# bwfbowen/muax

Hardware: AMD Instinct MI355X
Metric: batched act() env-steps/sec at num_simulations=50 (higher is better)
Workload: dtype f32; 1 GPU; cartpole: 4096 roots/GPU, obs 4, MLP embed 8, A=2, support 10, num_simulations=50, dirichlet 0.25/0.3, tiebreak=threefry, temperature 1; roots_per_gpu=4096, num_simulations=50, parallelism=roots sharded x1, no collective, backend=none (one rank), launcher=none

## Files before the change

### muax_amd/csrc/mz_fused.cuh

```cuda
#pragma once
#include "mz_spec.cuh"

#pragma clang fp contract(off)

namespace mz {

#ifdef MZ_PROFILE
#define MZ_TICK(slot)                                  \
  do {                                                 \
    uint64_t now_ = __builtin_amdgcn_s_memtime();      \
    prof_acc[slot] += now_ - prof_t;                   \
    prof_t = now_;                                     \
  } while (0)
#define MZ_TICKW(slot)                                 \
  do {                                                 \
    asm volatile("s_waitcnt vmcnt(0) lgkmcnt(0)" ::: "memory"); \
    MZ_TICK(slot);                                     \
  } while (0)
#else
#define MZ_TICK(slot) do {} while (0)
#define MZ_TICKW(slot) do {} while (0)
#endif

constexpr int kMaxSims = 256;
// ... 778 lines not shown
    for (int t = 0; t < C::ES; ++t) {
      int k = j + 16 * t;
      float acc = 0.0f;
      {
        const int kc = k < E ? k : 0;
        int i = 0;
        for (; i + 4 <= p.obs_dim; i += 4) {
          float o4[4], w4[4];
#pragma unroll
          for (int q = 0; q < 4; ++q) {
            o4[q] = ob[i + q];
            w4[q] = p.repr_w[(i + q) * E + kc];
          }
#pragma unroll
          for (int q = 0; q < 4; ++q) acc = __builtin_fmaf(o4[q], w4[q], acc);
        }
        for (; i < p.obs_dim; ++i) acc = __builtin_fmaf(ob[i], p.repr_w[i * E + kc], acc);
        acc = acc + p.repr_b[kc];
      }
      s[t] = k < E ? acc : 0.0f;
    }
    row_min_max_normalize<E>(s, j);
  }
  float v0, pl0;
  nets.predict(s, j, support, p.F, v0, pl0);
  uint32_t inv_bits = 0;
  if (p.invalid != nullptr) {
#pragma unroll
    for (int a = 0; a < A; ++a) inv_bits |= p.invalid[(size_t)r * A + a] ? (1u << a) : 0u;
  }
  int ncons = 0;
  int root_jw;
  {
    float lg, pq[1];
    if constexpr (!C::GUMBEL) {
      float x[1] = {pl0}, pr[1];
      row_softmax<A>(x, j, pr);
      float nz = (p.dirichlet_noise != nullptr && j < A) ? p.dirichlet_noise[(size_t)r * A + j] : 0.0f;
      float keep = 1.0f - p.dirichlet_fraction;
      float noisy = keep * pr[0] + p.dirichlet_fraction * nz;
      lg = log_pos(fmaxf(noisy, kFltTiny));
      if (p.invalid != nullptr) {
        float mx = row_max<4>(j < A ? lg : -INFINITY);
        lg = ((inv_bits >> j) & 1u) ? kFltLowest : lg - mx;
      }
      float lx[1] = {lg};
      row_softmax<A>(lx, j, pq);
    } else {
      lg = pl0;
      if (inv_bits != 0) {
        float mx = row_max<4>(j < A ? lg : -INFINITY);
        lg = ((inv_bits >> j) & 1u) ? kFltLowest : lg - mx;
      }
      pq[0] = 0.0f;
      float g;
      if (p.gumbel != nullptr) {
        g = j < A ? p.gumbel[(size_t)r * A + j] : 0.0f;
      } else {
        uint32_t x0, x1;
        bool second;
        bits_block(p.global_batch * (uint64_t)A, rg * (uint64_t)A + (uint64_t)(j < A ? j : 0), x0, x1, second);
        threefry2x32(p.k_gumbel[0], p.k_gumbel[1], x0, x1);
        g = p.gumbel_scale * gumbel_from_bits(second ? x1 : x0);
      }
      if (j < A) {
        tree[C::GUM0 + j] = g;
        tree[C::off_logit(j)] = lg;
      }
      ncons = min(p.max_considered, A - __builtin_popcount(inv_bits));
    }
    if (j < A) tree[C::off_prob(j)] = pq[0];
    if (ex && j < A) p.t_children_prior_logits[(size_t)r * N * A + j] = lg;
    if (j == 0) {
      itree[C::HDR0] = 1;
      tree[C::HDR0 + 1] = v0;
      if constexpr (C::RAW_OK) tree[C::HDR0 + 3] = v0;
      p.root_value[r] = v0;
      if (ex) p.t_raw_values[(size_t)r * N] = v0;
    }
#pragma unroll
    for (int t = 0; t < C::ES; ++t)
      if (j + 16 * t < E) {
        if constexpr (C::EMB_LDS) tree[C::EMB0 + j + 16 * t] = s[t];
        else gemb[j + 16 * t] = s[t];
      }
    float prob[A], val[A], rew[A], dis[A], sc[A];
    int vis[A];
#pragma unroll
    for (int a = 0; a < A; ++a) {
      prob[a] = tree[C::off_prob(a)];
      val[a] = 0.0f; vis[a] = 0; rew[a] = 0.0f; dis[a] = p.discount;
    }
    int cidx[A], best, child;
    bool safe;
    if constexpr (!C::GUMBEL) {
      float rcp1[A];
#pragma unroll
      for (int a = 0; a < A; ++a) rcp1[a] = 1.0f;
      puct_scores<A>(v0, tbl[2], prob, val, vis, rew, dis, rcp1, sc);
    } else {
      float logit[A], gum[A];
#pragma unroll
      for (int a = 0; a < A; ++a) {
        logit[a] = tree[C::off_logit(a)];
        gum[a] = tree[C::GUM0 + a];
      }
      gumbel_scores<A, C::QT>(true, v0, v0, logit, val, vis, rew, dis, gum, p.visit_table[(size_t)ncons * S],
                              inv_bits, sc);
    }
#pragma unroll
    for (int a = 0; a < A; ++a) {
      cidx[a] = -1;
      sc[a] = ((inv_bits >> a) & 1u) ? -INFINITY : sc[a];
    }
    decide<A, C::TB>(sc, cidx, best, child, safe);
    root_jw = jump_word(0, best, 0, !safe);
    if (j == 0) {
#pragma unroll
      for (int a = 0; a < A; ++a) tree[C::off_score(a)] = sc[a];
      itree[C::JUMP] = root_jw;
    }
  }

  int depth_total = 0;
  int pref_parent = 0;
  float pre[C::ES];
#pragma unroll
  for (int t = 0; t < C::ES; ++t) pre[t] = 0.0f;
  if constexpr (!C::EMB_LDS) {
#pragma unroll
    for (int t = 0; t < C::ES; ++t) pre[t] = s[t];
  }
  MZ_TICKW(12);

  for (int sim = 0; sim < S; ++sim) {
    MZ_TICK(0);
    int cv_next = 0;
    if constexpr (C::GUMBEL) cv_next = p.visit_table[(size_t)ncons * S + (sim + 1 < S ? sim + 1 : S - 1)];
    int parent, action, dP;
    int next = -1;
    parent = root_jw & 0xfff;
    action = (root_jw >> 12) & 0xf;
    dP = (root_jw >> 16) & 0xff;
    int depth = dP + 1;
    bool rare = depth > max_depth;
    if constexpr (C::TB) rare = rare || root_jw < 0;
    if (__builtin_amdgcn_ballot_w64(rare) != 0) {
      uint32_t fk0 = 0, fk1 = 0, fs0 = 0, fs1 = 0;
      int fk_level = -1;
      int jw = root_jw;
      for (;;) {
        parent = jw & 0xfff;
        action = (jw >> 12) & 0xf;
        dP = (jw >> 16) & 0xff;
        if constexpr (C::TB) {
          if (jw < 0 && dP + 1 <= max_depth) {
            const int* ndi = itree + __umul24((unsigned)parent, (unsigned)NS);
            if (fk_level < 0) {
              uint32_t x0, x1;
              bool second;
              bits_block(2 * p.global_batch, 2 * rg + (uint64_t)(j & 1), x0, x1, second);
              threefry2x32(p.sim_keys[sim][0], p.sim_keys[sim][1], x0, x1);
              uint32_t word = second ? x1 : x0;
              fk0 = bcast_u<0>(word);
              fk1 = bcast_u<1>(word);
              fk_level = 0;
            }
#ifdef MZ_PROFILE
            prof_acc[14] += 1;
            prof_acc[15] += (uint64_t)(dP + 1 - fk_level);
#endif
            while (fk_level <= dP) {
              uint32_t x0 = (uint32_t)(j & 1), x1 = 2u + (uint32_t)(j & 1);
              threefry2x32(fk0, fk1, x0, x1);
              fk0 = bcast_u<0>(x0); fk1 = bcast_u<1>(x0);
              fs0 = bcast_u<0>(x1); fs1 = bcast_u<1>(x1);
              fk_level += 1;
            }
            constexpr int NB = (A + 1) / 2;
            const int jb = j % NB;
            uint32_t x0 = (uint32_t)jb, x1 = (NB + jb < A) ? (uint32_t)(NB + jb) : 0u;
            threefry2x32(fs0, fs1, x0, x1);
            int cidx[A];
            float score[A];
            C::load_cidx(ndi, cidx);
            StaticFor<0, A>::run([&](auto ic) {
              constexpr int a = decltype(ic)::value;
              const uint32_t bits = bcast_u<(a % NB)>(a < NB ? x0 : x1);
              score[a] = __int_as_float(ndi[C::off_score(a)]) + 1e-7f * uniform_from_bits(bits);
            });
            int best = 0, bn = cidx[0];
            float bs = score[0];
#pragma unroll
            for (int a = 1; a < A; ++a) {
              bool take = score[a] > bs;
              bs = take ? score[a] : bs;
              best = take ? a : best;
              bn = take ? cidx[a] : bn;
            }
            action = best;
            next = bn;
            if (bn >= 0 && dP + 1 < max_depth) {
              jw = itree[__umul24((unsigned)bn, (unsigned)NS) + C::JUMP];
              next = -1;
              continue;
            }
          }
        }
        break;
      }
      depth = dP + 1;
      if (depth > max_depth) {
        depth = max_depth;
        const int* pb = C::PH ? gpath + (size_t)parent * C::PATHW : itree + __umul24((unsigned)parent, (unsigned)NS) + C::PATH0;
        const int e = depth - 1;
        const int ent = (pb[(e * C::ENTRY_BITS) >> 5] >> ((e * C::ENTRY_BITS) & 31)) & ((1 << C::ENTRY_BITS) - 1);
        parent = ent & ((1 << C::ENTRY_ACT_SHIFT) - 1);
        action = ent >> C::ENTRY_ACT_SHIFT;
        next = C::load_cidx1(itree + __umul24((unsigned)parent, (unsigned)NS), action);
      }
    }
    depth_total += depth;
    MZ_TICK(1);
    const bool fresh = next < 0;
    const int newn = fresh ? sim + 1 : next;

    float sp[C::ES];
#pragma unroll
    for (int t = 0; t < C::ES; ++t)
      if constexpr (C::EMB_LDS) {
        const int jc = j + 16 * t < E ? j + 16 * t : E - 1;
        const float v = tree[__umul24((unsigned)parent, (unsigned)NS) + C::EMB0 + jc];
        sp[t] = (j + 16 * t < E) ? v : 0.0f;
      } else {
        float v = pre[t];
        if (parent != pref_parent && j + 16 * t < E) v = gemb[(size_t)parent * E + j + 16 * t];
        sp[t] = (j + 16 * t < E) ? v : 0.0f;
      }
    float* nn = tree + __umul24((unsigned)newn, (unsigned)NS);
    int* nni = reinterpret_cast<int*>(nn);
    const unsigned po = __umul24((unsigned)parent, (unsigned)NS);
    const int vis_old = nni[C::HDR0];
    int ppw[C::PATHS];
#pragma unroll
    for (int t = 0; t < C::PATHS; ++t) {
      const int wi = j + 16 * t < C::PATHW ? j + 16 * t : 0;
      if constexpr (C::PH) ppw[t] = gpath[(size_t)parent * C::PATHW + wi];
      else ppw[t] = itree[po + C::PATH0 + wi];
    }
    float reward, value, pil, pprob;
    float ns[C::ES];
    nets.forward(sp, action, j, support, p.F, p.pred_on_parent != 0, reward, value, pil, pprob, ns);
    MZ_TICK(2);
    {
      const int vis = vis_old + 1;
      if (j < A) {
        nn[C::off_prob(j)] = pprob;
        if constexpr (C::GUMBEL) nn[C::off_logit(j)] = pil;
      }
#pragma unroll
      for (int t = 0; t < C::ES; ++t)
        if (j + 16 * t < E) {
          if constexpr (C::EMB_LDS) nn[C::EMB0 + j + 16 * t] = ns[t];
          else gemb[(size_t)newn * E + j + 16 * t] = ns[t];
        }
      if (j == 0) {
        nni[C::HDR0] = vis;
        nn[C::HDR0 + 1] = value;
        if constexpr (C::RAW_OK) nn[C::HDR0 + 3] = value;
        C::store_cidx(itree + po, action, newn);
        tree[po + C::off_rew(action)] = reward;
      }
      if (fresh) {
        const int e = depth - 1;
        const int sh = (e * C::ENTRY_BITS) & 31;
        const int ent = parent | (action << C::ENTRY_ACT_SHIFT);
#pragma unroll
        for (int t = 0; t < C::PATHS; ++t) {
          const int wi = j + 16 * t;
          int w = ppw[t];
          w = (wi == ((e * C::ENTRY_BITS) >> 5))
                  ? (int)(((unsigned)w & ~(((1u << C::ENTRY_BITS) - 1u) << sh)) | ((unsigned)ent << sh))
                  : w;
          if (wi < C::PATHW) {
            if constexpr (C::PH) gpath[(size_t)newn * C::PATHW + wi] = w;
            else nni[C::PATH0 + wi] = w;
          }
        }
      }
      if (ex) {
        size_t o = (size_t)r * N + newn;
        if (j < A) p.t_children_prior_logits[o * A + j] = pil;
        if (j == 0) {
          p.t_raw_values[o] = value;
          p.t_parents[o] = parent;
          p.t_action_from_parent[o] = action;
        }
      }
    }

    MZ_TICK(4);
    {
      int wmax;
      {
        const int d0 = __builtin_amdgcn_readlane(depth, 0), d1 = __builtin_amdgcn_readlane(depth, 16);
        const int d2 = __builtin_amdgcn_readlane(depth, 32), d3 = __builtin_amdgcn_readlane(depth, 48);
        int m01, m23;
        asm("s_max_i32 %0, %1, %2" : "=s"(m01) : "s"(d0), "s"(d1) : "scc");
        asm("s_max_i32 %0, %1, %2" : "=s"(m23) : "s"(d2), "s"(d3) : "scc");
        asm("s_max_i32 %0, %1, %2" : "=s"(wmax) : "s"(m01), "s"(m23) : "scc");
      }
      float G = value;
      float carry_v = value;
      int carry_n = -1;
      int carry_j = 0;
      for (int c = wmax >> 4; c >= 0; --c) {
        const int e = 16 * c + j;
        const bool valid = e <= depth;
        const bool isleaf = e == depth;
        const bool edge = e < depth;
        int pn, pa;
        {
          const int ec = e < depth - 1 ? e : 0;
          const int widx = (ec * C::ENTRY_BITS) >> 5;
          const int slot_c = ((16 * c * C::ENTRY_BITS) >> 5) >> 4;
          int psrc = ppw[0];
#pragma unroll
          for (int t = 1; t < C::PATHS; ++t) psrc = (slot_c == t) ? ppw[t] : psrc;
          const int pword = __builtin_amdgcn_ds_bpermute(4 * ((lane & ~15) + (widx & 15)), psrc);
          const int ent = (pword >> ((ec * C::ENTRY_BITS) & 31)) & ((1 << C::ENTRY_BITS) - 1);
          pn = ent & ((1 << C::ENTRY_ACT_SHIFT) - 1);
          pa = ent >> C::ENTRY_ACT_SHIFT;
          pn = e == depth - 1 ? parent : pn;
          pa = e == depth - 1 ? action : pa;
          pn = isleaf ? newn : pn;
          pa = isleaf ? 0 : pa;
          pn = valid ? pn : 0;
        }
        MZ_TICKW(6);
        float* nd = tree + __umul24((unsigned)pn, (unsigned)NS);
        int* ndi = reinterpret_cast<int*>(nd);
        const int cnt = ndi[C::HDR0];
        const float pv = nd[C::HDR0 + 1];
        float prob[A], val[A], rew[A], dis[A];
        int vis[A], cidx[A];
        C::load_cidx(ndi, cidx);
        C::load_vis(ndi, vis);
#pragma unroll
        for (int a = 0; a < A; ++a) {
          prob[a] = nd[C::off_prob(a)];
          val[a] = nd[C::off_val(a)];
          rew[a] = nd[C::off_rew(a)];
          dis[a] = p.discount;
        }
        int jch[A];
#pragma unroll
        for (int a = 0; a < A; ++a)
          jch[a] = itree[__umul24((unsigned)(cidx[a] < 0 ? 0 : cidx[a]), (unsigned)NS) + C::JUMP];
        const int nvis = edge ? cnt + 1 : cnt;
        const float2 tn_rc = *reinterpret_cast<const float2*>(tbl + 2 * (valid ? nvis : 0));
        float rcp1[A];
#pragma unroll
        for (int a = 0; a < A; ++a) {
          vis[a] = (edge && pa == a) ? vis[a] + 1 : vis[a];
          rcp1[a] = tbl[2 * (vis[a] + 1) + 1];
        }
        MZ_TICKW(7);
        float re = rew[0];
#pragma unroll
        for (int a = 1; a < A; ++a) re = (pa == a) ? rew[a] : re;
        re = edge ? re : 0.0f;
        const float ge = edge ? p.discount : 1.0f;
        const int kstart = min(15, wmax - 16 * c);
        float Gt = ge * G;
#define MZ_GSTEP_TXT "s_nop 1\n\tv_mul_f32_dpp %0, %1, %2 row_shl:1 row_mask:0xf bank_mask:0xf\n\tv_add_f32 %1, %0, %3\n\t"
#define MZ_GSTEP4 \
  asm volatile(MZ_GSTEP_TXT MZ_GSTEP_TXT MZ_GSTEP_TXT MZ_GSTEP_TXT : "+v"(Gt), "+v"(G) : "v"(ge), "v"(re));
        if (kstart >= 12) { MZ_GSTEP4 }
        if (kstart >= 8) { MZ_GSTEP4 }
        if (kstart >= 4) { MZ_GSTEP4 }
        float sc[A];
        constexpr bool kFill = !C::GUMBEL && A == 2;
        if constexpr (kFill) {
          float d0, d1, x0, x1, q0, q1, r0, r1;
#define MZ_GSTEP_BODY "v_mul_f32_dpp %[Gt], %[G], %[ge] row_shl:1 row_mask:0xf bank_mask:0xf\n\tv_add_f32 %[G], %[Gt], %[re]\n\t"
          asm volatile(
              "v_add_u32 %[d0], 1, %[v0]\n\tv_add_u32 %[d1], 1, %[v1]\n\tv_mul_f32 %[x0], %[tn], %[p0]\n\t" MZ_GSTEP_BODY
              "v_cvt_f32_i32 %[d0], %[d0]\n\tv_cvt_f32_i32 %[d1], %[d1]\n\tv_mul_f32 %[x1], %[tn], %[p1]\n\t" MZ_GSTEP_BODY
              "v_mul_f32 %[q0], %[x0], %[y0]\n\tv_mul_f32 %[q1], %[x1], %[y1]\n\tv_fma_f32 %[r0], -%[q0], %[d0], %[x0]\n\t" MZ_GSTEP_BODY
              "v_fma_f32 %[r1], -%[q1], %[d1], %[x1]\n\tv_fma_f32 %[s0], %[r0], %[y0], %[q0]\n\tv_fma_f32 %[s1], %[r1], %[y1], %[q1]\n\t"
              MZ_GSTEP_BODY
              : [Gt] "+v"(Gt), [G] "+v"(G), [d0] "=&v"(d0), [d1] "=&v"(d1), [x0] "=&v"(x0), [x1] "=&v"(x1), [q0] "=&v"(q0),
                [q1] "=&v"(q1), [r0] "=&v"(r0), [r1] "=&v"(r1), [s0] "=&v"(sc[0]), [s1] "=&v"(sc[A - 1])
              : [ge] "v"(ge), [re] "v"(re), [tn] "v"(tn_rc.x), [p0] "v"(prob[0]), [p1] "v"(prob[A - 1]), [v0] "v"(vis[0]),
                [v1] "v"(vis[A - 1]), [y0] "v"(rcp1[0]), [y1] "v"(rcp1[A - 1]));
#undef MZ_GSTEP_BODY
        } else {
          MZ_GSTEP4
        }
#undef MZ_GSTEP4
#undef MZ_GSTEP_TXT
        const float Gown = G;
        G = bcast<0>(G);
        MZ_TICKW(8);
        const float newv = div_small(pv * (float)cnt + Gown, (float)cnt + 1.0f, tn_rc.y);
        float childv = __int_as_float(__builtin_amdgcn_update_dpp(
            __float_as_int(carry_v), __float_as_int(newv), 0x101 , 0xf, 0xf, false));
        childv = (e == depth - 1) ? value : childv;
        carry_v = bcast<0>(newv);
        const int next_pn = __builtin_amdgcn_update_dpp(carry_n, pn, 0x101, 0xf, 0xf, false);
        carry_n = bcast_i<0>(pn);
#pragma unroll
        for (int a = 0; a < A; ++a) val[a] = (edge && pa == a) ? childv : val[a];
        const float nval = edge ? newv : pv;
        MZ_TICKW(9);
        if constexpr (!C::GUMBEL) {
          puct_scores<A, true, kFill>(nval, tn_rc.x, prob, val, vis, rew, dis, rcp1, sc);
#pragma unroll
          for (int a = 0; a < A; ++a)
            sc[a] = (pn == 0 && ((inv_bits >> a) & 1u)) ? -INFINITY : sc[a];
        } else {
          float logit[A], gum[A];
#pragma unroll
          for (int a = 0; a < A; ++a) {
            logit[a] = nd[C::off_logit(a)];
            gum[a] = tree[C::GUM0 + a];
          }
          gumbel_scores<A, C::QT>(pn == 0, nval, C::RAW_OK ? nd[C::HDR0 + C::HDRW - 1] : 0.0f, logit, val, vis, rew, dis, gum, cv_next,
                                  pn == 0 ? inv_bits : 0u, sc);
        }
        MZ_TICKW(10);
        int best, child;
        bool safe;
        decide<A, C::TB>(sc, cidx, best, child, safe);
        const bool inherit0 = valid && safe && child >= 0 && !isleaf && child == next_pn;
        int jchild = jch[0];
#pragma unroll
        for (int a = 1; a < A; ++a) jchild = (best == a) ? jch[a] : jchild;
        const int jwd0 = jump_word(pn, best, e, !safe);
        int jwd = (safe && child >= 0 && !inherit0) ? jchild : jwd0;
        int done = inherit0 ? 0 : -1;
#define MZ_JSCAN(d)                                                                              \
  {                                                                                              \
    const int jn = __builtin_amdgcn_update_dpp(0, jwd, 0x100 + d, 0xf, 0xf, true);               \
    const int dn = __builtin_amdgcn_update_dpp(0, done, 0x100 + d, 0xf, 0xf, true);              \
    jwd = (jwd & done) | (jn & ~done);                                                           \
    done = done | dn;                                                                            \
  }
        MZ_JSCAN(1) MZ_JSCAN(2) MZ_JSCAN(4) MZ_JSCAN(8)
#undef MZ_JSCAN
        jwd = (jwd & done) | (carry_j & ~done);
        carry_j = bcast_i<0>(jwd);
        MZ_TICKW(11);
        if (valid) {
#pragma unroll
          for (int a = 0; a < A; ++a) nd[C::off_score(a)] = sc[a];
          ndi[C::JUMP] = jwd;
          ndi[C::HDR0] = nvis;
          nd[C::HDR0 + 1] = nval;
          float cvn = val[0];
          int cin = vis[0];
#pragma unroll
          for (int a = 1; a < A; ++a) {
            cvn = (pa == a) ? val[a] : cvn;
            cin = (pa == a) ? vis[a] : cin;
          }
          nd[C::off_val(pa)] = cvn;
          C::store_vis(ndi, pa, cin);
        }
      }
      root_jw = carry_j;
      if constexpr (!C::EMB_LDS) {
        pref_parent = carry_j & 0xfff;
#pragma unroll
        for (int t = 0; t < C::ES; ++t)
          pre[t] = (j + 16 * t < E) ? gemb[(size_t)pref_parent * E + j + 16 * t] : 0.0f;
      }
    }
    MZ_TICK(5);
  }

  if constexpr (C::GUMBEL) {
    float logit[A], val[A], rew[A], dis[A], gum[A], qv[A], sc[A], x[A], w[A];
    int vis[A], sumv, cv = 0;
#pragma unroll
    for (int a = 0; a < A; ++a) {
      val[a] = tree[C::off_val(a)];
      vis[a] = itree[C::ST0 + C::STW * a + 2];
      rew[a] = tree[C::off_rew(a)];
      dis[a] = p.discount;
      logit[a] = tree[C::off_logit(a)];
      gum[a] = tree[C::GUM0 + a];
      cv = max(cv, vis[a]);
    }
    const float nval = tree[C::HDR0 + 1], raw = C::RAW_OK ? tree[C::HDR0 + C::HDRW - 1] : 0.0f;
    gumbel_scores<A, C::QT>(true, nval, raw, logit, val, vis, rew, dis, gum, cv, inv_bits, sc);
    qtransform_inlane<A, C::QT>(nval, raw, logit, val, vis, rew, dis, qv, sumv);
    int best = 0;
    float bs = sc[0], mx = logit[0] + qv[0];
#pragma unroll
    for (int a = 0; a < A; ++a) {
      x[a] = logit[a] + qv[a];
      mx = fmaxf(mx, x[a]);
      bool take = a > 0 && sc[a] > bs;
      bs = take ? sc[a] : bs;
      best = take ? a : best;
    }
    if (inv_bits != 0) {
#pragma unroll
      for (int a = 0; a < A; ++a) x[a] = ((inv_bits >> a) & 1u) ? kFltLowest : x[a] - mx;
    }
    softmax_inlane<A>(x, w);
    if (j < A) {
      float mine = w[0];
#pragma unroll
      for (int a = 1; a < A; ++a) mine = (j == a) ? w[a] : mine;
      p.action_weights[(size_t)r * A + j] = mine;
    }
    if (j == 0) {
      p.action[r] = best;
      if (p.search_value) p.search_value[r] = nval;
      if (p.depth_sum) p.depth_sum[r] = depth_total;
    }
  } else {
  {
    const int ja = j < A ? j : A - 1;
    int vc;
    if constexpr (C::PK) vc = reinterpret_cast<const uint8_t*>(itree + C::VIS0)[ja];
    else vc = itree[C::ST0 + C::STW * ja + 2];
    vc = j < A ? vc : 0;
    float total = (float)row_sum_i(vc);
    float denom = fmaxf(total, 1.0f);
    float prob = (float)vc / denom;
    prob = total > 0.0f ? prob : 1.0f / (float)A;
    float lg = log_pos(fmaxf(prob, kFltTiny));
    float mx = row_max<4>(j < A ? lg : -INFINITY);
    float tden = fmaxf(p.temperature, kFltTiny);
    float al = (lg - mx) / tden;
    float g;
    if (p.gumbel != nullptr) {
      g = j < A ? p.gumbel[(size_t)r * A + j] : 0.0f;
    } else {
      uint32_t x0, x1;
      bool second;
      bits_block(p.global_batch * (uint64_t)A, rg * (uint64_t)A + (uint64_t)ja, x0, x1, second);
      threefry2x32(p.k_sample[0], p.k_sample[1], x0, x1);
      g = gumbel_from_bits(second ? x1 : x0);
    }
    float score = j < A ? al + g : -INFINITY;
    int best = j, dummy = 0;
    row_argmax<4>(score, best, dummy);
    if (j < A) p.action_weights[(size_t)r * A + j] = prob;
    if (j == 0) {
      p.action[r] = best;
      if (p.search_value) p.search_value[r] = tree[C::HDR0 + 1];
      if (p.depth_sum) p.depth_sum[r] = depth_total;
    }
  }
  }

  if (ex) {
    for (int n = 0; n < N; ++n) {
      size_t o = (size_t)r * N + n;
      const float* nd = tree + n * NS;
      const int* ndi = itree + n * NS;
      if (j == 0) {
        p.t_node_visits[o] = ndi[C::HDR0];
        p.t_node_values[o] = nd[C::HDR0 + 1];
      }
      if (j < A) {
        int ci, cv;
        if constexpr (C::PK) {
          ci = reinterpret_cast<const int8_t*>(ndi + C::SEL0)[j];
          cv = reinterpret_cast<const uint8_t*>(ndi + C::VIS0)[j];
        } else {
          ci = ndi[C::SEL0 + 2 * j];
          cv = ndi[C::ST0 + C::STW * j + 2];
        }
        p.t_children_index[o * A + j] = ci;
        p.t_children_values[o * A + j] = nd[C::off_val(j)];
        p.t_children_visits[o * A + j] = cv;
        p.t_children_rewards[o * A + j] = nd[C::off_rew(j)];
        p.t_children_discounts[o * A + j] = ci >= 0 ? p.discount : 0.0f;
      }
      if constexpr (C::EMB_LDS)
        for (int i = j; i < E; i += 16) p.t_embeddings[o * E + i] = nd[C::EMB0 + i];
    }
  }
  MZ_TICKW(13);
#ifdef MZ_PROFILE
  if (p.prof != nullptr && lane == 0) {
    uint64_t* dst = p.prof + ((size_t)blockIdx.x * C::WAVES + (tid >> 6)) * 16;
    for (int q = 0; q < 16; ++q) dst[q] = prof_acc[q];
  }
#endif
}

}
```

Baseline: 34.93 million env-steps/s.

## Pack four roots' backup paths into one wave-wide pass when depths fit

Adds a wide backup mode. When the four 16-lane roots in a wave have total path length up to 64 and the max depth is at least 16, their path nodes are laid across the whole wave and backed up in a single pass. This uses wave_shl DPP for the discounted return scan and readlane-based carry of jump words, replacing multiple 16-lane chunk iterations. It adds readlane/select overhead and per-lane root remapping, and only applies when PATHS==1, so deep trees with multiple chunks benefit while shallow ones take the old path.

```diff
diff --git a/muax_amd/csrc/mz_fused.cuh b/muax_amd/csrc/mz_fused.cuh
--- a/muax_amd/csrc/mz_fused.cuh
+++ b/muax_amd/csrc/mz_fused.cuh
@@ -1104,20 +1104,25 @@
     MZ_TICK(4);
     {
       int wmax;
+      const int dep0 = __builtin_amdgcn_readlane(depth, 0), dep1 = __builtin_amdgcn_readlane(depth, 16);
+      const int dep2 = __builtin_amdgcn_readlane(depth, 32), dep3 = __builtin_amdgcn_readlane(depth, 48);
       {
-        const int d0 = __builtin_amdgcn_readlane(depth, 0), d1 = __builtin_amdgcn_readlane(depth, 16);
-        const int d2 = __builtin_amdgcn_readlane(depth, 32), d3 = __builtin_amdgcn_readlane(depth, 48);
         int m01, m23;
-        asm("s_max_i32 %0, %1, %2" : "=s"(m01) : "s"(d0), "s"(d1) : "scc");
-        asm("s_max_i32 %0, %1, %2" : "=s"(m23) : "s"(d2), "s"(d3) : "scc");
+        asm("s_max_i32 %0, %1, %2" : "=s"(m01) : "s"(dep0), "s"(dep1) : "scc");
+        asm("s_max_i32 %0, %1, %2" : "=s"(m23) : "s"(dep2), "s"(dep3) : "scc");
         asm("s_max_i32 %0, %1, %2" : "=s"(wmax) : "s"(m01), "s"(m23) : "scc");
       }
+      constexpr bool kWideBackup = !C::PH && C::PATHS == 1 && A <= 16;
+      const int woff1 = dep0 + 1, woff2 = woff1 + dep1 + 1, woff3 = woff2 + dep2 + 1;
       float G = value;
       float carry_v = value;
       int carry_n = -1;
       int carry_j = 0;
-      for (int c = wmax >> 4; c >= 0; --c) {
-        const int e = 16 * c + j;
+      auto backup_pass = [&](auto wide_c, const int c, float* const tree, const int e, const int depth, const int parent,
+                             const int action, const int newn, const float value, const uint32_t inv_bits,
+                             const int cv_next, const int psrc, const int srcrow) {
+        constexpr bool WIDE = decltype(wide_c)::value;
+        int* const itree = reinterpret_cast<int*>(tree);
         const bool valid = e <= depth;
         const bool isleaf = e == depth;
         const bool edge = e < depth;
@@ -1125,11 +1130,7 @@
         {
           const int ec = e < depth - 1 ? e : 0;
           const int widx = (ec * C::ENTRY_BITS) >> 5;
-          const int slot_c = ((16 * c * C::ENTRY_BITS) >> 5) >> 4;
-          int psrc = ppw[0];
-#pragma unroll
-          for (int t = 1; t < C::PATHS; ++t) psrc = (slot_c == t) ? ppw[t] : psrc;
-          const int pword = __builtin_amdgcn_ds_bpermute(4 * ((lane & ~15) + (widx & 15)), psrc);
+          const int pword = __builtin_amdgcn_ds_bpermute(4 * (srcrow + (widx & 15)), psrc);
           const int ent = (pword >> ((ec * C::ENTRY_BITS) & 31)) & ((1 << C::ENTRY_BITS) - 1);
           pn = ent & ((1 << C::ENTRY_ACT_SHIFT) - 1);
           pa = ent >> C::ENTRY_ACT_SHIFT;
@@ -1172,46 +1173,59 @@
 #pragma unroll
         for (int a = 1; a < A; ++a) re = (pa == a) ? rew[a] : re;
         re = edge ? re : 0.0f;
-        const float ge = edge ? p.discount : 1.0f;
-        const int kstart = min(15, wmax - 16 * c);
+        float ge = edge ? p.discount : 1.0f;
+        if constexpr (WIDE) {
+          re = isleaf ? value : re;
+          ge = isleaf ? 0.0f : ge;
+        }
+        if constexpr (WIDE) G = value;
         float Gt = ge * G;
-#define MZ_GSTEP_TXT "s_nop 1\n\tv_mul_f32_dpp %0, %1, %2 row_shl:1 row_mask:0xf bank_mask:0xf\n\tv_add_f32 %1, %0, %3\n\t"
-#define MZ_GSTEP4 \
-  asm volatile(MZ_GSTEP_TXT MZ_GSTEP_TXT MZ_GSTEP_TXT MZ_GSTEP_TXT : "+v"(Gt), "+v"(G) : "v"(ge), "v"(re));
-        if (kstart >= 12) { MZ_GSTEP4 }
-        if (kstart >= 8) { MZ_GSTEP4 }
-        if (kstart >= 4) { MZ_GSTEP4 }
+#define MZ_GSTEP_TXT(SHL) "s_nop 1\n\tv_mul_f32_dpp %0, %1, %2 " SHL " row_mask:0xf bank_mask:0xf\n\tv_add_f32 %1, %0, %3\n\t"
+#define MZ_GSTEP4(SHL) \
+  asm volatile(MZ_GSTEP_TXT(SHL) MZ_GSTEP_TXT(SHL) MZ_GSTEP_TXT(SHL) MZ_GSTEP_TXT(SHL) : "+v"(Gt), "+v"(G) : "v"(ge), "v"(re));
+        if constexpr (WIDE) {
+          for (int k = wmax >> 2; k > 0; --k) { MZ_GSTEP4("wave_shl:1") }
+        } else {
+          const int kstart = min(15, wmax - 16 * c);
+          if (kstart >= 12) { MZ_GSTEP4("row_shl:1") }
+          if (kstart >= 8) { MZ_GSTEP4("row_shl:1") }
+          if (kstart >= 4) { MZ_GSTEP4("row_shl:1") }
+        }
         float sc[A];
         constexpr bool kFill = !C::GUMBEL && A == 2;
         if constexpr (kFill) {
           float d0, d1, x0, x1, q0, q1, r0, r1;
-#define MZ_GSTEP_BODY "v_mul_f32_dpp %[Gt], %[G], %[ge] row_shl:1 row_mask:0xf bank_mask:0xf\n\tv_add_f32 %[G], %[Gt], %[re]\n\t"
-          asm volatile(
-              "v_add_u32 %[d0], 1, %[v0]\n\tv_add_u32 %[d1], 1, %[v1]\n\tv_mul_f32 %[x0], %[tn], %[p0]\n\t" MZ_GSTEP_BODY
-              "v_cvt_f32_i32 %[d0], %[d0]\n\tv_cvt_f32_i32 %[d1], %[d1]\n\tv_mul_f32 %[x1], %[tn], %[p1]\n\t" MZ_GSTEP_BODY
-              "v_mul_f32 %[q0], %[x0], %[y0]\n\tv_mul_f32 %[q1], %[x1], %[y1]\n\tv_fma_f32 %[r0], -%[q0], %[d0], %[x0]\n\t" MZ_GSTEP_BODY
-              "v_fma_f32 %[r1], -%[q1], %[d1], %[x1]\n\tv_fma_f32 %[s0], %[r0], %[y0], %[q0]\n\tv_fma_f32 %[s1], %[r1], %[y1], %[q1]\n\t"
-              MZ_GSTEP_BODY
-              : [Gt] "+v"(Gt), [G] "+v"(G), [d0] "=&v"(d0), [d1] "=&v"(d1), [x0] "=&v"(x0), [x1] "=&v"(x1), [q0] "=&v"(q0),
-                [q1] "=&v"(q1), [r0] "=&v"(r0), [r1] "=&v"(r1), [s0] "=&v"(sc[0]), [s1] "=&v"(sc[A - 1])
-              : [ge] "v"(ge), [re] "v"(re), [tn] "v"(tn_rc.x), [p0] "v"(prob[0]), [p1] "v"(prob[A - 1]), [v0] "v"(vis[0]),
-                [v1] "v"(vis[A - 1]), [y0] "v"(rcp1[0]), [y1] "v"(rcp1[A - 1]));
+#define MZ_GSTEP_BODY(SHL) "v_mul_f32_dpp %[Gt], %[G], %[ge] " SHL " row_mask:0xf bank_mask:0xf\n\tv_add_f32 %[G], %[Gt], %[re]\n\t"
+#define MZ_GFILL4(SHL)                                                                                                            \
+  asm volatile(                                                                                                                   \
+      "v_add_u32 %[d0], 1, %[v0]\n\tv_add_u32 %[d1], 1, %[v1]\n\tv_mul_f32 %[x0], %[tn], %[p0]\n\t" MZ_GSTEP_BODY(SHL)              \
+      "v_cvt_f32_i32 %[d0], %[d0]\n\tv_cvt_f32_i32 %[d1], %[d1]\n\tv_mul_f32 %[x1], %[tn], %[p1]\n\t" MZ_GSTEP_BODY(SHL)            \
+      "v_mul_f32 %[q0], %[x0], %[y0]\n\tv_mul_f32 %[q1], %[x1], %[y1]\n\tv_fma_f32 %[r0], -%[q0], %[d0], %[x0]\n\t" MZ_GSTEP_BODY(SHL) \
+      "v_fma_f32 %[r1], -%[q1], %[d1], %[x1]\n\tv_fma_f32 %[s0], %[r0], %[y0], %[q0]\n\tv_fma_f32 %[s1], %[r1], %[y1], %[q1]\n\t"   \
+      MZ_GSTEP_BODY(SHL)                                                                                                          \
+      : [Gt] "+v"(Gt), [G] "+v"(G), [d0] "=&v"(d0), [d1] "=&v"(d1), [x0] "=&v"(x0), [x1] "=&v"(x1), [q0] "=&v"(q0),               \
+        [q1] "=&v"(q1), [r0] "=&v"(r0), [r1] "=&v"(r1), [s0] "=&v"(sc[0]), [s1] "=&v"(sc[A - 1])                                  \
+      : [ge] "v"(ge), [re] "v"(re), [tn] "v"(tn_rc.x), [p0] "v"(prob[0]), [p1] "v"(prob[A - 1]), [v0] "v"(vis[0]),                \
+        [v1] "v"(vis[A - 1]), [y0] "v"(rcp1[0]), [y1] "v"(rcp1[A - 1]));
+          if constexpr (WIDE) { MZ_GFILL4("wave_shl:1") } else { MZ_GFILL4("row_shl:1") }
+#undef MZ_GFILL4
 #undef MZ_GSTEP_BODY
         } else {
-          MZ_GSTEP4
+          if constexpr (WIDE) { MZ_GSTEP4("wave_shl:1") } else { MZ_GSTEP4("row_shl:1") }
         }
 #undef MZ_GSTEP4
 #undef MZ_GSTEP_TXT
         const float Gown = G;
-        G = bcast<0>(G);
+        if constexpr (!WIDE) G = bcast<0>(G);
         MZ_TICKW(8);
         const float newv = div_small(pv * (float)cnt + Gown, (float)cnt + 1.0f, tn_rc.y);
+        constexpr int kShl1 = WIDE ? 0x130  : 0x101 ;
         float childv = __int_as_float(__builtin_amdgcn_update_dpp(
-            __float_as_int(carry_v), __float_as_int(newv), 0x101 , 0xf, 0xf, false));
+            __float_as_int(carry_v), __float_as_int(newv), kShl1, 0xf, 0xf, false));
         childv = (e == depth - 1) ? value : childv;
-        carry_v = bcast<0>(newv);
-        const int next_pn = __builtin_amdgcn_update_dpp(carry_n, pn, 0x101, 0xf, 0xf, false);
-        carry_n = bcast_i<0>(pn);
+        if constexpr (!WIDE) carry_v = bcast<0>(newv);
+        const int next_pn = __builtin_amdgcn_update_dpp(carry_n, pn, kShl1, 0xf, 0xf, false);
+        if constexpr (!WIDE) carry_n = bcast_i<0>(pn);
 #pragma unroll
         for (int a = 0; a < A; ++a) val[a] = (edge && pa == a) ? childv : val[a];
         const float nval = edge ? newv : pv;
@@ -1251,8 +1265,20 @@
   }
         MZ_JSCAN(1) MZ_JSCAN(2) MZ_JSCAN(4) MZ_JSCAN(8)
 #undef MZ_JSCAN
-        jwd = (jwd & done) | (carry_j & ~done);
-        carry_j = bcast_i<0>(jwd);
+        if constexpr (!WIDE) {
+          jwd = (jwd & done) | (carry_j & ~done);
+          carry_j = bcast_i<0>(jwd);
+        } else {
+          const int drow = lane >> 4;
+#pragma unroll
+          for (int q = 2; q >= 0; --q) {
+            const int cj = __builtin_amdgcn_readlane(jwd, 16 * (q + 1));
+            jwd = (drow == q && done == 0) ? cj : jwd;
+          }
+          const int w0 = __builtin_amdgcn_readlane(jwd, 0), w1 = __builtin_amdgcn_readlane(jwd, woff1);
+          const int w2 = __builtin_amdgcn_readlane(jwd, woff2), w3 = __builtin_amdgcn_readlane(jwd, woff3);
+          carry_j = drow == 0 ? w0 : drow == 1 ? w1 : drow == 2 ? w2 : w3;
+        }
         MZ_TICKW(11);
         if (valid) {
 #pragma unroll
@@ -1269,6 +1295,39 @@
           }
           nd[C::off_val(pa)] = cvn;
           C::store_vis(ndi, pa, cin);
+        }
+      };
+      bool wide = false;
+      if constexpr (kWideBackup) wide = wmax >= 16 && woff3 + dep3 + 1 <= 64;
+      if (wide) {
+        if constexpr (kWideBackup) {
+          const bool q1 = lane >= woff1, q2 = lane >= woff2, q3 = lane >= woff3;
+          auto sel = [&](int x0, int x1, int x2, int x3) {
+            int x = q1 ? x1 : x0;
+            x = q2 ? x2 : x;
+            return q3 ? x3 : x;
+          };
+          auto pick = [&](int x) {
+            return sel(__builtin_amdgcn_readlane(x, 0), __builtin_amdgcn_readlane(x, 16), __builtin_amdgcn_readlane(x, 32),
+                       __builtin_amdgcn_readlane(x, 48));
+          };
+          const unsigned pk = (unsigned)pick((int)((unsigned)parent | ((unsigned)action << 12) | ((unsigned)depth << 16) | ((unsigned)newn << 24)));
+          const int q16 = sel(0, 16, 32, 48);
+          float* const wtree = tree - (lane >> 4) * C::ROOT_WORDS + sel(0, C::ROOT_WORDS, 2 * C::ROOT_WORDS, 3 * C::ROOT_WORDS);
+          int cvn = 0;
+          if constexpr (C::GUMBEL) cvn = pick(cv_next);
+          backup_pass(std::true_type{}, 0, wtree, lane - sel(0, woff1, woff2, woff3), (int)((pk >> 16) & 0xffu),
+                      (int)(pk & 0xfffu), (int)((pk >> 12) & 0xfu), (int)(pk >> 24), __int_as_float(pick(__float_as_int(value))),
+                      (uint32_t)pick((int)inv_bits), cvn, ppw[0], q16);
+        }
+      } else {
+        for (int c = wmax >> 4; c >= 0; --c) {
+          const int slot_c = ((16 * c * C::ENTRY_BITS) >> 5) >> 4;
+          int psrc = ppw[0];
+#pragma unroll
+          for (int t = 1; t < C::PATHS; ++t) psrc = (slot_c == t) ? ppw[t] : psrc;
+          backup_pass(std::false_type{}, c, tree, 16 * c + j, depth, parent, action, newn, value, inv_bits, cv_next, psrc,
+                      lane & ~15);
         }
       }
       root_jw = carry_j;
```

Result: faster. 35.43 million env-steps/s, median of 6 (+1.4%).
